# konstin/knn-for-homology

Measured on AMD Instinct MI355X. Metric: queries/sec, flat inner-product kNN, d=1024 fp32, k=100 (recall@k = 1.0: exact flat search), higher is better.
Workload: dtype f32; 1 GPU; BASELINE configs[3]: synthetic 10000000x1024 fp32 flat IP, k=100, 32 queries per step, DB row-sharded over 1 GPU(s); nb_total=10000000, nb_per_gpu=10000000, d=1024, k=100, parallelism=db-row-shard x1, searches_in_flight=1

## Files before the change

### knn-for-homology_amd/csrc/knn355.hip

```cpp
#include <hip/hip_runtime.h>
#include <thread>
#include <type_traits>
#include <stdint.h>
#include <stdio.h>
#include <string.h>
#include <float.h>
#include <math.h>
#include <algorithm>
#include <mutex>
#include <condition_variable>
#include <chrono>
#include <memory>
#include <atomic>
#include <string>
#include <vector>

#include "../../include/knn355.h"
#include "plan.h"

typedef float f32x4 __attribute__((ext_vector_type(4)));
typedef float f32x2 __attribute__((ext_vector_type(2)));
typedef float f32x16 __attribute__((ext_vector_type(16)));
typedef const __attribute__((address_space(1))) f32x4 *gptr4;
typedef __bf16 bf16x8 __attribute__((ext_vector_type(8)));
// ... 868 lines not shown
    "v_cmp_le_f32_e64 %[m0], %[t0], %[e0]\n\t" "v_cmp_le_f32_e64 %[m1], %[t1], %[e1]\n\t" "v_cmp_le_f32_e64 %[m2], %[t2], %[e2]\n\t" "v_cmp_le_f32_e64 %[m3], %[t3], %[e3]\n\t"
#define KNN_P1_TAIL "v_min_u32_e32 %[ad0], %[w], %[dump]\n\t" "v_cndmask_b32_e64 %[u], 0, %[step], %[m0]\n\t" "v_add_u32_e32 %[w], %[w], %[u]\n\t" \
    "v_min_u32_e32 %[ad1], %[w], %[dump]\n\t" "v_cndmask_b32_e64 %[u], 0, %[step], %[m1]\n\t" "v_add_u32_e32 %[w], %[w], %[u]\n\t" \
    "v_min_u32_e32 %[ad2], %[w], %[dump]\n\t" "v_cndmask_b32_e64 %[u], 0, %[step], %[m2]\n\t" "v_add_u32_e32 %[w], %[w], %[u]\n\t" \
    "v_min_u32_e32 %[ad3], %[w], %[dump]\n\t" "v_cndmask_b32_e64 %[u], 0, %[step], %[m3]\n\t" "v_add_u32_e32 %[w], %[w], %[u]\n\t" \
    "v_mov_b32_e32 %[i0], %[idx0]\n\t" "v_mov_b32_e32 %[i1], %[idx1]\n\t" "v_mov_b32_e32 %[i2], %[idx2]\n\t" "v_mov_b32_e32 %[i3], %[idx3]\n\t" \
    "ds_write2_b32 %[ad0], %[t0], %[i0] offset1:1\n\t" "ds_write2_b32 %[ad1], %[t1], %[i1] offset1:1\n\t" "ds_write2_b32 %[ad2], %[t2], %[i2] offset1:1\n\t" "ds_write2_b32 %[ad3], %[t3], %[i3] offset1:1"
#define KNN_P1_OUT_ROW , [e0] "=&v"(e[0]), [e1] "=&v"(e[1]), [e2] "=&v"(e[2]), [e3] "=&v"(e[3])
#define KNN_P1_IN_L2 , [s0] "v"(s0), [s1] "v"(s1), [s2] "v"(s2), [s3] "v"(s3)
#define KNN_P1_IN_THR , [thr] "v"(thr[b])
#define KNN_P1_IN_ROW , [h0] "v"(t2l[sc - c + 0]), [h1] "v"(t2l[sc - c + 1]), [h2] "v"(t2l[sc - c + 2]), [h3] "v"(t2l[sc - c + 3]), [ninf] "v"(ninf), [cok] "s"(cokm[b])
#define KNN_PASS1(head, bound, out_bound, acc_reg, in_l2, in_bound) asm volatile(head bound KNN_P1_TAIL \
    : [t0] "=&v"(t[0]), [t1] "=&v"(t[1]), [t2] "=&v"(t[2]), [t3] "=&v"(t[3]), [ad0] "=&v"(ad[0]), [ad1] "=&v"(ad[1]), [ad2] "=&v"(ad[2]), [ad3] "=&v"(ad[3]), [i0] "=&v"(ix[0]), [i1] "=&v"(ix[1]), [i2] "=&v"(ix[2]), [i3] "=&v"(ix[3]), [m0] "=&s"(mk[0]), [m1] "=&s"(mk[1]), [m2] "=&s"(mk[2]), [m3] "=&s"(mk[3]), [u] "=&v"(u), [w] "+v"(w) out_bound \
    : [a0] acc_reg(a0), [a1] acc_reg(a1), [a2] acc_reg(a2), [a3] acc_reg(a3) in_l2 in_bound, [dump] "v"(dump), [step] "v"(step), [idx0] "n"((sc + 0) | (b << 8)), [idx1] "n"((sc + 1) | (b << 8)), [idx2] "n"((sc + 2) | (b << 8)), [idx3] "n"((sc + 3) | (b << 8)) : "memory")

template <int WM, int WN, int TM, int TN, bool L2, bool NTDB = false, bool SYM = false, bool BF16 = false, int DNQ = 0, int Q16 = 0, bool F16X = false, bool X12 = false>
__global__ __launch_bounds__(256, (TM * TN >= 16 ? 1 : 2)) void flat_scan_kernel(ScanParams p)
{
    if (p.gate) {
        uint32_t any = 0;
        for (int i = 0; i < p.gate_n; i++) any |= p.gate[i];
        if (!any) return;
    }
    constexpr bool DIFF = DNQ > 0;
    static_assert(!F16X || (NTDB && !L2 && !SYM && !BF16 && DNQ == 0 && Q16 == 0 && TN == 1), "the 16-bit prefilter: one query tile, inner product");
    static_assert(!X12 || (F16X && WM == 4 && TM == 2), "the 12-bit row copies: the prefilter's 256-row tile");
    constexpr bool H16 = BF16 || F16X;
    static_assert(WM * WN == 4, "4 waves per workgroup");
    static_assert(!DIFF || (L2 && !SYM && !BF16 && WN == 1 && TN == 1), "the difference build: one 32-query tile, squared L2");
    constexpr bool M16 = Q16 > 0;
    static_assert(!M16 || (NTDB && !SYM && !BF16 && DNQ == 0 && TN == 1), "16-query blocks: plain fp32, one query tile per launch");
    constexpr int DT = WM * TM * 32;
    constexpr int QT = WN * (M16 ? Q16 * 16 : TN * 32);
    constexpr int NB = M16 ? Q16 : TN;
    constexpr int NS = TM * (M16 ? 8 : 16);
    constexpr bool BIGT = TM * TN >= 16;
    constexpr bool SPARSE = !NTDB && !BF16 && DNQ == 0 && Q16 == 0 && WM == 2 && WN == 2 && TM == TN && (TM == 2 || TM == 4);
    constexpr int ROWS = DT + QT;
    constexpr int X12_DB = 24;
    constexpr int NGRP = X12 ? X12_DB + QT / 8 : ROWS / 8;
    constexpr int NI = (NGRP + 3) / 4;
    static_assert(ROWS % 8 == 0, "staging split");
    static_assert(!X12 || NGRP % 4 == 0, "X12: every wave issues whole rounds, the last of them the queries'");
    constexpr int NDBI = X12 ? X12_DB / 4 : DT / 32;
    constexpr int KOFF_DB = X12 ? X12_DB * 256 : 32;
    constexpr int B_OFF = X12 ? X12_DB * 1024 : DT * 128;
    constexpr int STAGE_BYTES = ROWS * 128;
    extern __shared__ __attribute__((aligned(16))) char smem[];
    char *stage0 = smem;
    char *stage1 = smem + STAGE_BYTES;
    const int lds_main = max(max(2 * STAGE_BYTES, p.cap * 8), SYM && TM * TN == 4 ? 73728 : 0);

    const int tid = threadIdx.x;
    const int lane = tid & 63;
// ... 312 lines not shown
                    if constexpr (t < 3) __builtin_amdgcn_sched_group_barrier(0x100, RT + Q16, 0);
                    constexpr int nd = n1 - n0, per = M / (nd + 1);
                    static_assert(per >= 1, "more staging instructions than MFMAs in a sub-step");
                    sched_spread<nd, per>();
                    __builtin_amdgcn_sched_group_barrier(0x008, M - nd * per, 0);
                };
                substep16(std::integral_constant<int, 0>{});
                substep16(std::integral_constant<int, 1>{});
                substep16(std::integral_constant<int, 2>{});
                substep16(std::integral_constant<int, 3>{});
                return;
            }
            if constexpr (X12) {
                typedef uint32_t u32x4 __attribute__((ext_vector_type(4)));
                typedef _Float16 f16x2 __attribute__((ext_vector_type(2)));
                u32x4 hi[TM][2], lo[TM];
                f32x4 bq[4][TN];
#pragma unroll
                for (int a = 0; a < TM; a++) {
                    hi[a][0] = *(const u32x4 *)(A + ((wm * TM + a) * 2 + 0) * 1024 + lane * 16);
                    hi[a][1] = *(const u32x4 *)(A + ((wm * TM + a) * 2 + 1) * 1024 + lane * 16);
                    lo[a] = *(const u32x4 *)(A + DT * 64 + (wm * TM + a) * 1024 + lane * 16);
                }
#pragma unroll
                for (int t = 0; t < 4; t++)
#pragma unroll
                    for (int b = 0; b < TN; b++) bq[t][b] = *(const f32x4 *)(B + ((wn * TN + b) * 32 + li) * 128 + (((2 * t + lh) ^ swz) * 16));
#pragma unroll
                for (int n = 0; n < ND; n++) dma(n);
                const f16x2 bias = {(_Float16)1216.0f, (_Float16)1216.0f}, sixteen = {(_Float16)16.0f, (_Float16)16.0f};
                auto pair = [&](uint32_t hw, uint32_t lw, uint32_t sel) -> uint32_t {
                    const f16x2 ah = __builtin_bit_cast(f16x2, __builtin_amdgcn_perm(0x64646464u, hw, sel)) - bias;
                    const f16x2 al = __builtin_bit_cast(f16x2, __builtin_amdgcn_perm(0x64646464u, lw, sel));
                    return __builtin_bit_cast(uint32_t, __builtin_elementwise_fma(ah, sixteen, al));
                };
#pragma unroll
                for (int t = 0; t < 4; t++) {
#pragma unroll
                    for (int a = 0; a < TM; a++) {
                        const uint32_t h0 = hi[a][t >> 1][2 * (t & 1)], h1 = hi[a][t >> 1][2 * (t & 1) + 1];
                        const uint32_t l0 = lo[a][t] & 0x0F0F0F0Fu, l1 = (lo[a][t] >> 4) & 0x0F0F0F0Fu;
                        const u32x4 fr = {pair(h0, l0, 0x04010400u), pair(h0, l0, 0x04030402u), pair(h1, l1, 0x04010400u), pair(h1, l1, 0x04030402u)};
#pragma unroll
                        for (int b = 0; b < TN; b++)
                            acc[a][b] = __builtin_amdgcn_mfma_f32_32x32x16_f16(__builtin_bit_cast(f16x8, fr), __builtin_bit_cast(f16x8, bq[t][b]), acc[a][b], 0, 0, 0);
                    }
                }
                return;
            }
            f32x4 af[2][TM], bf[2][TN];
            auto frag = [&](int t) {
                const int slot = ((2 * t + lh) ^ swz) * 16;
#pragma unroll
                for (int a = 0; a < TM; a++)
                    af[t & 1][a] = *(const f32x4 *)(A + ((wm * TM + a) * 32 + li) * 128 + slot);
#pragma unroll
                for (int b = 0; b < TN; b++)
// ... 1120 lines not shown
    bool bad;
    const int e = s16_convert(xb + (size_t)r * dp, dp, dp16, xs + (size_t)r * dp16, -128, lane, &nx, &nxp, &nd, &bad);
    if (lane == 0) {
        xexp[r] = (int8_t)e;
        if (bad) {
            atomicOr(&stat[S16_NONFINITE], 1u);
        } else {
            atomicMax(&stat[S16_R], __float_as_uint(s16_up(nd)));
            atomicMax(&stat[S16_XP], __float_as_uint(s16_up(nxp)));
            atomicMax(&stat[S16_X], __float_as_uint(s16_up(nx)));
            atomicMax((int *)&stat[S16_EMAX], e);
        }
    }
}

__global__ __launch_bounds__(256) void scan12_rows_kernel(const float *__restrict__ xb, int dp, int64_t r0, int64_t n, int dp16,
                                                          uint8_t *__restrict__ xs, int8_t *__restrict__ xexp, uint32_t *__restrict__ stat)
{
    const int lane = threadIdx.x & 63;
    const int64_t r = r0 + (int64_t)blockIdx.x * 4 + (threadIdx.x >> 6);
    if (r >= r0 + n) return;
    const float *x = xb + (size_t)r * dp;
    float mx = 0.0f;
    bool nf = false;
    for (int i = lane; i < dp; i += 64) {
        const float v = x[i];
        nf |= !isfinite(v);
        mx = fmaxf(mx, fabsf(v));
    }
    for (int o = 32; o > 0; o >>= 1) mx = fmaxf(mx, __shfl_xor(mx, o, 64));
    const bool bad = __ballot(nf) != 0ull;
    int e = (mx > 0.0f && isfinite(mx)) ? ilogbf(mx) - 10 : 0;
    e = max(e, -128);
    const int KT = dp16 / 64, rt = (int)(r & 255), li = rt & 31, wa = rt >> 5;
    uint8_t *tile = xs + (size_t)(r >> 8) * KT * 24576;
    double sx = 0.0, sxp = 0.0, sd = 0.0;
    for (int g = lane; g < dp16 / 8; g += 64) {
        const int ks = g >> 3, t = (g >> 1) & 3, lh = g & 1;
        uint32_t hw[2] = {0u, 0u}, lw = 0u;
        for (int j = 0; j < 8; j++) {
            const int i = 8 * g + j;
            const float v = i < dp ? x[i] : 0.0f;
            float nv = rintf(ldexpf(v, -e));
            nv = fminf(fmaxf(nv, -2047.0f), 2047.0f);
            const int ni = nv == nv ? (int)nv : 0;
            const uint32_t u = (uint32_t)(ni + 2048);
            hw[j >> 2] |= (u >> 4) << (8 * (j & 3));
            lw |= (u & 15u) << (8 * (j & 3) + 4 * (j >> 2));
            const double xp = ldexp((double)ni, e), dv = (double)v;
            sx += dv * dv;
            sxp += xp * xp;
            sd += (dv - xp) * (dv - xp);
        }
        uint8_t *ksp = tile + (size_t)ks * 24576;
        *(uint2 *)(ksp + (wa * 2 + (t >> 1)) * 1024 + (lh * 32 + li) * 16 + (t & 1) * 8) = make_uint2(hw[0], hw[1]);
        *(uint32_t *)(ksp + 16384 + wa * 1024 + (lh * 32 + li) * 16 + t * 4) = lw;
    }
    for (int o = 32; o > 0; o >>= 1) {
        sx += __shfl_xor(sx, o, 64);
        sxp += __shfl_xor(sxp, o, 64);
        sd += __shfl_xor(sd, o, 64);
    }
    if (lane == 0) {
        xexp[r] = (int8_t)e;
        if (bad) {
            atomicOr(&stat[S16_NONFINITE], 1u);
        } else {
            atomicMax(&stat[S16_R], __float_as_uint(s16_up(sqrt(sd))));
            atomicMax(&stat[S16_XP], __float_as_uint(s16_up(sqrt(sxp))));
            atomicMax(&stat[S16_X], __float_as_uint(s16_up(sqrt(sx))));
            atomicMax((int *)&stat[S16_EMAX], e);
// ... 370 lines not shown
};

struct knn_index_s {
    int d = 0, dp = 0, metric = 0, device = 0;
    int num_cus = 256;
    int64_t ntotal = 0, cap_rows = 0;
    bool is_view = false;
    std::shared_ptr<std::atomic<int64_t>> storage_gen = std::make_shared<std::atomic<int64_t>>(0);
    int64_t view_gen = 0;
    float *xb = nullptr;
    bool approx16 = false;
    bool keep16 = false;
    DevBuf xb16, ws_q16;
    int scan16 = 0;
    int s16_fmt = 16;
    std::shared_ptr<std::atomic<bool>> s16_ok = std::make_shared<std::atomic<bool>>(false);
    int dp16 = 0;
    DevBuf s16_rows_buf, s16_exp_buf, s16_stat_buf;
    const _Float16 *s16_rows = nullptr;
    const int8_t *s16_exp = nullptr;
    const uint32_t *s16_stat = nullptr;
    std::string s16_note;
    DevBuf ws_q16x, ws_s16q, ws_s16ak, ws_s16ok, ws_s16stat;
    bool last_s16_used = false;
    int last_s16_fmt = 0;
    int s16_pieces = 0;
    float *yn = nullptr;
    size_t xb_bytes = 0, yn_bytes = 0;
    hipStream_t stream = nullptr;
    hipEvent_t done = nullptr;
// ... 210 lines not shown
    (void)hipEventCreateWithFlags(&h->done, hipEventDisableTiming);
    *out = h;
    return 0;
}

static void free_index_buffers(knn_index_s *h)
{
    if (!h->is_view) h->storage_gen->fetch_add(1);
    if (h->xb && !h->is_view) g_pool.give(h->xb, h->xb_bytes, h->device);
    if (h->yn && !h->is_view) g_pool.give(h->yn, h->yn_bytes, h->device);
    if (!h->is_view) {
        h->s16_rows_buf.release();
        h->s16_exp_buf.release();
        h->s16_stat_buf.release();
        if (h->scan16 == 2) h->scan16 = 1;
    }
    h->s16_rows = nullptr;
    h->s16_exp = nullptr;
    h->s16_stat = nullptr;
    if (!h->is_view) h->s16_ok->store(false);
    h->xb = nullptr;
    h->yn = nullptr;
    h->ntotal = 0;
    h->cap_rows = 0;
}

extern "C" void knn_free(knn_handle h)
{
    if (!h) return;
    if (hipSetDevice(h->device) == hipSuccess) {
// ... 88 lines not shown
    if (h->xb16.bytes < need) {
        if (h->xb16.ensure(need)) return set_err(KNN_ERR_HIP, "add: out of device memory (bf16 rows)");
        n += r0;
        r0 = 0;
    }
    const int64_t total = n * h->dp;
    const unsigned grid = (unsigned)std::min<int64_t>((total / 4 + 255) / 256, 65535);
    hipLaunchKernelGGL(to_bf16_kernel, dim3(grid), dim3(256), 0, s, h->xb + (size_t)r0 * h->dp, total, (__bf16 *)h->xb16.p + (size_t)r0 * h->dp);
    HIP_TRY(hipGetLastError());
    return 0;
}

static int scan16_sync_rows(knn_index_s *h, int64_t r0, int64_t n, hipStream_t s)
{
    if (h->scan16 != 1 || h->is_view) return 0;
    const size_t need = h->s16_fmt == 12 ? (size_t)((h->cap_rows + 255) / 256) * (h->dp16 / 64) * 24576 : (size_t)h->cap_rows * h->dp16 * 2;
    if (h->cap_rows > 0 && (h->s16_rows_buf.bytes < need || h->s16_exp_buf.bytes < (size_t)h->cap_rows || !h->s16_stat_buf.p)) {
        HIP_TRY(hipStreamSynchronize(s));
        if (h->s16_rows_buf.p || h->s16_exp_buf.p) {
            h->storage_gen->fetch_add(1);
            (void)hipDeviceSynchronize();
        }
        if (h->s16_rows_buf.ensure(need) || h->s16_exp_buf.ensure((size_t)h->cap_rows) || h->s16_stat_buf.ensure(S16_NSTAT * 4)) {
            h->s16_rows_buf.release();
            h->s16_exp_buf.release();
            h->s16_stat_buf.release();
            h->s16_rows = nullptr;
            h->s16_exp = nullptr;
            h->s16_stat = nullptr;
            h->s16_ok->store(false);
            h->scan16 = 2;
            h->s16_note = "dropped: no device memory for the row copies";
            return 0;
        }
        n += r0;
        r0 = 0;
    }
    if (n <= 0) return 0;
    h->s16_rows = (const _Float16 *)h->s16_rows_buf.p;
    h->s16_exp = (const int8_t *)h->s16_exp_buf.p;
    h->s16_stat = (const uint32_t *)h->s16_stat_buf.p;
    uint32_t init[S16_NSTAT] = {0u, 0u, 0u, 0x80000000u, 0u, 0u, 0u, 0u};
    if (r0 == 0) HIP_TRY(hipMemcpyAsync(h->s16_stat_buf.p, init, sizeof init, hipMemcpyHostToDevice, s));
    if (h->s16_fmt == 12)
        hipLaunchKernelGGL(scan12_rows_kernel, dim3((unsigned)((n + 3) / 4)), dim3(256), 0, s, h->xb, h->dp, r0, n, h->dp16,
                           (uint8_t *)h->s16_rows_buf.p, (int8_t *)h->s16_exp_buf.p, (uint32_t *)h->s16_stat_buf.p);
    else
        hipLaunchKernelGGL(scan16_rows_kernel, dim3((unsigned)((n + 3) / 4)), dim3(256), 0, s, h->xb, h->dp, r0, n, h->dp16,
                           (_Float16 *)h->s16_rows_buf.p, (int8_t *)h->s16_exp_buf.p, (uint32_t *)h->s16_stat_buf.p);
    HIP_TRY(hipGetLastError());
    uint32_t nonfinite = 0;
    HIP_TRY(hipMemcpyAsync(&nonfinite, (const uint32_t *)h->s16_stat_buf.p + S16_NONFINITE, 4, hipMemcpyDeviceToHost, s));
    HIP_TRY(hipStreamSynchronize(s));
    h->s16_ok->store(nonfinite == 0);
    h->s16_note = nonfinite ? "off: a row holds a value that is not finite" : "on";
    return 0;
}

static int flat_set_approx16(knn_index_s *h)
{
// ... 199 lines not shown
}

static ScanKernel pick_scan_kernel(int qt, bool l2, bool approx16, bool one_qtile, int diff_width, int pass_mode, int s16_fmt = 16)
{
    if (const char *why = scan_kernel_illegal(qt, l2, approx16, one_qtile, pass_mode)) {
        set_err(KNN_ERR_INVALID, why);
        return nullptr;
    }
    switch (qt) {
    case 256: return l2 ? flat_scan_kernel<2, 2, 4, 4, true, false> : flat_scan_kernel<2, 2, 4, 4, false, false>;
    case 128: return scan_build<2, 2, 2, 2>(l2, approx16, one_qtile);
    case 96: return l2 ? flat_scan_kernel<2, 2, 2, 1, true, true, false, false, 0, 3> : flat_scan_kernel<2, 2, 2, 1, false, true, false, false, 0, 3>;
    case 48: return l2 ? flat_scan_kernel<4, 1, 2, 1, true, true, false, false, 0, 3> : flat_scan_kernel<4, 1, 2, 1, false, true, false, false, 0, 3>;
    case 64: return scan_build<2, 2, 2, 1>(l2, approx16, one_qtile);
    }
    if (pass_mode == 1 && s16_fmt == 12) return flat_scan_kernel<4, 1, 2, 1, false, true, false, false, 0, 0, true, true>;
    if (pass_mode == 1) return flat_scan_kernel<4, 1, 2, 1, false, true, false, false, 0, 0, true>;
    switch (diff_width) {
    case 0: break;
    case 8: return flat_scan_kernel<4, 1, 2, 1, true, true, false, false, 8>;
    case 12: return flat_scan_kernel<4, 1, 2, 1, true, true, false, false, 12>;
    case 16: return flat_scan_kernel<4, 1, 2, 1, true, true, false, false, 16>;
    default: return flat_scan_kernel<4, 1, 2, 1, true, true, false, false, 20>;
    }
    return scan_build<4, 1, 2, 1>(l2, approx16, one_qtile);
}

static ScanKernel pick_sym_kernel(int ts, bool l2)
{
    if (ts == 128) return l2 ? flat_scan_kernel<2, 2, 2, 2, true, false, true> : flat_scan_kernel<2, 2, 2, 2, false, false, true>;
    return l2 ? flat_scan_kernel<2, 2, 4, 4, true, false, true> : flat_scan_kernel<2, 2, 4, 4, false, false, true>;
// ... 156 lines not shown
    }
    if (pl.npairs && sstride) {
        if (lb.pair_ctr.ensure(((size_t)pl.npairs + 1) * 4, h->done, s)) return set_err(KNN_ERR_HIP, "search: out of device memory");
        HIP_TRY(hipMemsetD32Async((hipDeviceptr_t)lb.pair_ctr.p, 2, (size_t)pl.npairs, s));
        HIP_TRY(hipMemsetD32Async((hipDeviceptr_t)((uint32_t *)lb.pair_ctr.p + pl.npairs), 0, 1, s));
    }
    if (h->ws_lists.ensure((size_t)pl.grid * pl.qt * pl.cap * 8, h->done, s)) return set_err(KNN_ERR_HIP, "search: out of device memory (candidate lists)");
    ScanParams p = {};
    p.xb = h->xb; p.yn = h->yn; p.xq = q_dev; p.xn = xn;
    p.nb = nb; p.nq = nq; p.dp = h->dp; p.k = k; p.cap = pl.cap;
    if (h->approx16) {
        p.xb = (const float *)h->xb16.p;
        p.dp = h->dp / 2;
    }
    if (pass.mode == 1) {
        if (h->s16_fmt == 12 && (row_mul != 1 || sstride)) return set_err(KNN_ERR_INVALID, "search: the 12-bit row copies cannot serve a strided view");
        p.xb = (const float *)h->s16_rows;
        p.dp = h->dp16 / 2;
        p.xexp = h->s16_exp;
        p.qexp = pass.qexp;
    }
    p.gate = pass.gate;
    p.gate_n = pass.gate_n;
    p.nqtiles = pl.nqtiles; p.nchunks = pl.nchunks; p.tiles_base = pl.tiles_base; p.tiles_rem = pl.tiles_rem;
    p.lists = (uint64_t *)h->ws_lists.p; p.gthr = gthr;
    p.qlist = qlist; p.qcnt = qcnt; p.qcap = qcap;
    p.id_base = id_base;
    p.row_mul = row_mul;
    p.vshift = sstride ? svshift : vshift;
    p.skip_mask = sstride ? sstride - 1 : -1;
    p.kslot = plan.kslot;
// ... 25 lines not shown
        if (g_trace_buf.ensure((size_t)pl.grid * 128 * 8)) return set_err(KNN_ERR_HIP, "trace: out of device memory");
        HIP_TRY(hipMemsetAsync(g_trace_buf.p, 0, (size_t)pl.grid * 128 * 8, s));
        p.trace = (unsigned long long *)g_trace_buf.p;
        p.ablate = getenv("KNN355_ABLATE") ? atoi(getenv("KNN355_ABLATE")) : 0;
        g_trace_grid = pl.grid;
    }
#endif
    if (top && (rc = open_timed_launch(h, s))) return rc;
    const ScanKernel kern = pick_scan_kernel(pl.qt, h->metric == KNN_METRIC_L2, h->approx16, pl.nqtiles == 1, pl.diff ? diff_build_width(nq) : 0, pass.mode, h->s16_fmt);
    if (!kern) return KNN_ERR_INVALID;
    rc = scan_lds_opt_in(kern, pl.lds);
    if (!rc) rc = launch_scan(kern, p, pl.grid, pl.lds, s);
    if (rc) return rc;
    if (top) {
        HIP_TRY(hipEventRecord(h->ev1, s));
        h->last_kernel = pass.mode == 1 ? std::string(pl.name) + (h->s16_fmt == 12 ? "_x12" : "_f16x") : std::string(pl.name); h->last_qt = pl.qt; h->last_dt = pl.dt; h->last_chunks = pl.nchunks; h->last_grid = pl.grid;
        h->last_seed_stride = pub_rounds ? -pub_rounds * pub_m : sstride;
        h->last_seed_stat = seed_stat ? plan.seed_j : 0;
        h->last_sample_rows = sstride ? view_rows(nb, sstride, p.vshift) : 0;
    }
    SelectParams sp = {};
    sp.in = qlist; sp.in_stride = qcap; sp.cnt = qcnt; sp.cap = qcap;
    sp.n_expect = select_expect_n(plan, nb, k, sstride ? view_rows(nb, sstride, p.vshift) : 0);
    sp.nq = nq; sp.k = k; sp.metric = h->metric;
    sp.out_keys = out.keys; sp.out_stride = out.keys ? out.keys_stride : 0; sp.out_fill = out.keys_fill;
    sp.D = out.D; sp.I = out.I;
    sp.seed_cnt = out.seed_cnt; sp.seed_gthr = out.seed_gthr; sp.seed_qthr = out.seed_qthr; sp.seed_j = out.seed_j; sp.seed_stat = out.seed_stat;
    sp.seed_nslots = out.seed_nslots;
    sp.qthr = qthr; sp.fail = (int *)h->ws_flag.p;
    sp.gate = pass.gate; sp.gate_n = pass.gate_n; sp.gate_count = pass.gate_count;
    if (reset_sig && out.seed_cnt == nullptr) {
// ... 672 lines not shown
extern "C" int knn_flat_reserve(knn_handle h, int64_t nrows)
{
    if (!h) return set_err(KNN_ERR_INVALID, "reserve: null handle");
    if (nrows < 0 || nrows > 0xFFFFFFF0ll) return set_err(KNN_ERR_INVALID, "reserve: bad row count");
    std::lock_guard<std::mutex> lk(h->mu);
    if (h->is_view) return set_err(KNN_ERR_INVALID, "reserve: a view is read-only");
    HIP_TRY(hipSetDevice(h->device));
    if (nrows <= h->cap_rows) return 0;
    if (int rc = move_storage(h, nrows, "reserve")) return rc;
    return scan16_sync_rows(h, h->ntotal, 0, h->stream);
}

extern "C" int knn_flat_set_scan16(knn_handle h, int32_t mode)
{
    if (!h) return set_err(KNN_ERR_INVALID, "set_scan16: null handle");
    if (mode != 0 && mode != 1 && mode != 2) return set_err(KNN_ERR_INVALID, "set_scan16: mode must be 0, 1 or 2");
    std::lock_guard<std::mutex> lk(h->mu);
    if (h->is_view) return set_err(KNN_ERR_INVALID, "set_scan16: a view uses its parent's setting");
    if (mode && (h->approx16 || h->keep16)) return set_err(KNN_ERR_UNSUPPORTED, "set_scan16: not for an index that keeps bf16 copies (HNSW)");
    if (h->ntotal != 0) return set_err(KNN_ERR_INVALID, "set_scan16: the index already holds rows");
    const char *env = getenv("KNN355_SCAN16");
    if (mode && env && strcmp(env, "0") == 0) mode = 0;
    const char *fenv = getenv("KNN355_SCAN_FORMAT");
    if (mode == 2 && fenv && strcmp(fenv, "16") == 0) mode = 1;
    h->scan16 = mode ? 1 : 0;
    h->s16_fmt = mode == 2 ? 12 : 16;
    h->dp16 = round_up(h->d, 64);
    h->s16_note = mode ? "on" : "off";
    return 0;
}

extern "C" int knn_last_scan16_info(knn_handle h, int32_t *used, int32_t *candidates_max, int64_t *fallbacks)
{
    if (!h) return set_err(KNN_ERR_INVALID, "null handle");
    std::lock_guard<std::mutex> lk(h->mu);
    uint32_t st[2] = {0u, 0u};
    if (h->ws_s16stat.p) {
        HIP_TRY(hipSetDevice(h->device));
        HIP_TRY(hipDeviceSynchronize());
        HIP_TRY(hipMemcpy(st, h->ws_s16stat.p, sizeof st, hipMemcpyDeviceToHost));
    }
// ... 414 lines not shown
```

### knn-for-homology_amd/csrc/plan.h

```cpp
#pragma once
#include <stddef.h>
#include <stdint.h>
#include <stdlib.h>
#include <math.h>
#include <algorithm>
#include <vector>

#include "../../include/knn355.h"

struct PlanCtx {
    int metric = KNN_METRIC_INNER_PRODUCT;
    bool approx16 = false;
    int flags = 0, force_qt = 0, force_chunks = 0;
    int num_cus = 256;
    int64_t batch_nq = 0;
    int pub_rounds_force = 0;
    int64_t ntotal = 0;
    int s16_fmt = 16;
};

static inline int64_t view_rows(int64_t n, int row_mul, int vshift)
{
    const int64_t B = (int64_t)1 << vshift, span = B * row_mul;
    if (n <= 0) return 0;
// ... 142 lines not shown
{
    if (S < 64 || N <= 0 || k >= N) return -1;
    const double pr = (double)k / (double)N, eps = 1e-9;
    const double lp = log(pr), lq = log1p(-pr);
    double cdf = 0.0;
    const int64_t jmax = std::min<int64_t>(S, k);
    for (int64_t i = 0; i <= jmax; i++) {
        if (1.0 - cdf <= eps) return i >= 1 ? (int)i : 1;
        cdf += exp(lgamma((double)S + 1.0) - lgamma((double)i + 1.0) - lgamma((double)(S - i) + 1.0) + (double)i * lp + (double)(S - i) * lq);
    }
    return -1;
}

static int s16_kprime(int k, int fmt = 16)
{
    if (fmt == 12) return std::min(KNN_WAVE_SELECT_MAX_K, std::max(3 * k, k + 128));
    return std::min(KNN_WAVE_SELECT_MAX_K, std::max(2 * k, k + 64));
}

static bool s16_eligible(const PlanCtx &c, int pass_mode, int64_t nb, int64_t nq, int k, int row_mul, int level, int dp, int fmt = 16)
{
    if (pass_mode || level != 0 || row_mul != 1) return false;
    if (c.metric != KNN_METRIC_INNER_PRODUCT || c.approx16 || (c.flags & KNN_TUNE_NO_SCAN16)) return false;
    if (nq < 1 || nq > 32 || (c.force_qt != 0 && c.force_qt != 32) || s16_kprime(k, fmt) <= k) return false;
    if ((size_t)dp * 4 + 64 > 65536) return false;
    return nb >= (1 << 18) || (c.flags & KNN_TUNE_SCAN16_ANY_NB);
}

struct SearchPlan {
    ScanPlan pl;
    int sstride;
    int svshift;
    int seed_j, seed_stat, k_sample;
    int pub_rounds, pub_m;
    int kslot, qcap;
    double expect_n;
    int pool_tiles;
    bool sparse_epi, cu_turn;
};
// ... 54 lines not shown
        if (c.pub_rounds_force > 0 && (int64_t)c.pub_rounds_force * pl.nchunks <= 2048 && c.pub_rounds_force < pl.tiles_base &&
            (int64_t)c.pub_rounds_force * pl.nchunks >= (int64_t)k + 32)
            pub_rounds = c.pub_rounds_force;
    }
    if (!pub_rounds && pub_shape && !c.pub_rounds_force && nb >= 16 * (int64_t)k && k <= KNN_WAVE_SELECT_MAX_K) {
        const int wm = (pl.qt == 32 || pl.qt == 48) ? 4 : 2;
        for (int r = 2; r >= 1; r--) {
            const int64_t P = (int64_t)r * wm * pl.nchunks;
            if (P <= 4096 && P >= (int64_t)k + k / 4 + 32 && r < pl.tiles_base) {
                pub_rounds = r;
                pub_m = wm;
            }
        }
    }
    if (pass_mode == 2 && !pub_rounds) sstride = 0;
    if (pass_mode == 1 && c.s16_fmt == 12 && !pub_rounds) sstride = 0;
    if (pub_rounds) {
        sstride = 0;
        expect_n = 2.0 * (double)k * (double)nb / ((double)pub_rounds * pl.nchunks * pl.dt) + 2.0 * k + 64;
        if (pub_m > 1) {
            const double P = (double)pub_rounds * pub_m * pl.nchunks;
            expect_n = 1.3 * (-P * log(1.0 - (double)k / P)) * (double)nb / ((double)pub_rounds * pl.nchunks * pl.dt) + 2.0 * k + 64;
        }
    }
    if (!sstride && !pub_rounds) {
        PlanOpts final_plan;
        final_plan.seeded = level > 0; final_plan.allow_pairs = allow_pairs && level == 0; final_plan.allow_big = allow_big;
        make_plan(c, nb, nq, k, final_plan, pl);
    }
    int kslot = knn_kslot(k);
    if (pl.chunk_rows == pl.dt && pl.dt > kslot && pl.dt <= pl.cap - pl.dt && k <= KNN_WAVE_SELECT_MAX_K) kslot = pl.dt;
// ... 459 lines not shown
```

### knn-for-homology_amd/csrc/plan_check.cpp

```cpp
#include "plan.h"

#include <stdarg.h>
#include <stdio.h>
#include <string.h>
#include <set>
#include <string>
#include <tuple>

static const int MAX_LEVELS = 8;

static PlanCtx make_ctx(int64_t nb, int64_t nq, int metric, int flags, int force_qt, int force_chunks, int64_t batch, bool approx16)
{
    PlanCtx c;
    c.metric = metric;
    c.approx16 = approx16;
    c.flags = flags & ~KNN_TUNE_PUB_ROUNDS_MASK;
    c.pub_rounds_force = (flags & KNN_TUNE_PUB_ROUNDS_MASK) >> KNN_TUNE_PUB_ROUNDS_SHIFT;
    c.force_qt = force_qt;
    c.force_chunks = force_chunks;
    c.num_cus = 256;
    c.batch_nq = batch > 0 ? std::max(nq, batch) : nq;
    c.ntotal = nb;
    return c;
}
// ... 437 lines not shown
        starts.push_back(starts[0]);
        stops.push_back(stops[0]);
        for (int64_t chunk_rows : {(int64_t)1, (int64_t)2, (int64_t)7, (int64_t)64, (int64_t)119, (int64_t)120, rows - 1, rows, rows + 1, (int64_t)1 << 40})
            if (chunk_rows >= 1) check_pool_chunks(starts, stops, chunk_rows);
    }
}

static int run_s16()
{
    long long nb, nq;
    int k, flags;
    while (scanf("%lld %lld %d %d", &nb, &nq, &k, &flags) == 4) {
        const PlanCtx c = make_ctx(nb, nq, KNN_METRIC_INNER_PRODUCT, flags, 0, 0, 0, false);
        printf("%lld %lld %d %d: fp16 kprime %d eligible %d, 12-bit kprime %d eligible %d\n", nb, nq, k, flags, s16_kprime(k, 16),
               (int)s16_eligible(c, 0, nb, nq, k, 1, 0, 1024, 16), s16_kprime(k, 12), (int)s16_eligible(c, 0, nb, nq, k, 1, 0, 1024, 12));
    }
    return 0;
}

static int run_sweep()
{
    const int64_t nbs[] = {1, 255, 256, 257, 1023, 4096, 8192, 16385, 1 << 15, 1 << 18, (1 << 18) + 1, 1250000, 10000000, 2147483647};
    const int64_t nqs[] = {1, 8, 19, 20, 32, 33, 48, 49, 64, 65, 96, 97, 128, 129, 256, 384, 640, 16384, 24576, 24577, 200000};
    const int ks[] = {1, 10, 100, 301, 1000, 1400, 1401, 2048};
    const int flagset[] = {0, KNN_TUNE_NO_POOL, KNN_TUNE_NO_PAIRS, KNN_TUNE_NO_SEED, KNN_TUNE_EXACT_SEED, KNN_TUNE_NORM_L2, KNN_TUNE_ALWAYS_RESET,
                           KNN_TUNE_STAT_SEED, KNN_TUNE_NO_TURNS, KNN_TUNE_NO_STAT_SEED, KNN_TUNE_NO_SYM, KNN_TUNE_NO_TILE_MIN_SEED,
                           1 << KNN_TUNE_PUB_ROUNDS_SHIFT, 2 << KNN_TUNE_PUB_ROUNDS_SHIFT, KNN_TUNE_NO_REMAINDER_SPLIT, KNN_TUNE_NO_Q16,
                           KNN_TUNE_NO_BIG_TILE, KNN_TUNE_BIG_TILE, KNN_TUNE_NO_SCAN16, KNN_TUNE_SCAN16_ANY_NB};
    const int qts[] = {0, 32, 48, 64, 96, 128, 256};
    for (int64_t nb : nbs)
// ... 28 lines not shown
                for (int key_bytes : {2, 4, 8})
                    for (int outs = 0; outs < 8; outs++) check_rank(rows, k, limit, key_bytes, outs);
        }
    sweep_pool();
    sweep_kde();
    printf("plan_check sweep: %lld plans checked, %lld broken\n", g_checked, g_broken);
    return g_broken ? 1 : 0;
}

int main(int argc, char **argv)
{
    if (argc == 2 && !strcmp(argv[1], "cases")) return run_cases();
    if (argc == 2 && !strcmp(argv[1], "sym")) return run_sym();
    if (argc == 2 && !strcmp(argv[1], "range")) return run_range();
    if (argc == 2 && !strcmp(argv[1], "s16")) return run_s16();
    if (argc == 2 && !strcmp(argv[1], "rank")) return run_rank();
    if (argc == 2 && !strcmp(argv[1], "pool")) return run_pool();
    if (argc == 2 && !strcmp(argv[1], "poolchunks")) return run_poolchunks();
    if (argc == 2 && !strcmp(argv[1], "kde")) return run_kde();
    if (argc == 2 && !strcmp(argv[1], "sweep")) return run_sweep();
    fprintf(stderr, "usage: plan_check cases|sym|range|s16|rank|pool|poolchunks|kde < lines | plan_check sweep\n");
    return 2;
}
```

Before: 12750 queries/s.

## Add 10-bit packed row copies for the prefilter scan, auto-selected on large indexes

Adds a 10-bit packed format for the database copies used by the 16-bit prefilter pass, alongside the existing 12-bit one. A byte high part plus 2-bit low parts cut each k-step tile from 24 KiB to 20 KiB. The point is to reduce the memory bandwidth of the bandwidth-bound scan. Mode 2 now picks 10-bit automatically when rows×dims reach 2^33 values. The cost is coarser quantisation, so the candidate count k' grows to max(8k, k+256), which adds selection work and exact rescoring.

```diff
diff --git a/knn-for-homology_amd/csrc/knn355.hip b/knn-for-homology_amd/csrc/knn355.hip
--- a/knn-for-homology_amd/csrc/knn355.hip
+++ b/knn-for-homology_amd/csrc/knn355.hip
@@ -906,7 +906,7 @@
     : [t0] "=&v"(t[0]), [t1] "=&v"(t[1]), [t2] "=&v"(t[2]), [t3] "=&v"(t[3]), [ad0] "=&v"(ad[0]), [ad1] "=&v"(ad[1]), [ad2] "=&v"(ad[2]), [ad3] "=&v"(ad[3]), [i0] "=&v"(ix[0]), [i1] "=&v"(ix[1]), [i2] "=&v"(ix[2]), [i3] "=&v"(ix[3]), [m0] "=&s"(mk[0]), [m1] "=&s"(mk[1]), [m2] "=&s"(mk[2]), [m3] "=&s"(mk[3]), [u] "=&v"(u), [w] "+v"(w) out_bound \
     : [a0] acc_reg(a0), [a1] acc_reg(a1), [a2] acc_reg(a2), [a3] acc_reg(a3) in_l2 in_bound, [dump] "v"(dump), [step] "v"(step), [idx0] "n"((sc + 0) | (b << 8)), [idx1] "n"((sc + 1) | (b << 8)), [idx2] "n"((sc + 2) | (b << 8)), [idx3] "n"((sc + 3) | (b << 8)) : "memory")
 
-template <int WM, int WN, int TM, int TN, bool L2, bool NTDB = false, bool SYM = false, bool BF16 = false, int DNQ = 0, int Q16 = 0, bool F16X = false, bool X12 = false>
+template <int WM, int WN, int TM, int TN, bool L2, bool NTDB = false, bool SYM = false, bool BF16 = false, int DNQ = 0, int Q16 = 0, bool F16X = false, int XW = 0>
 __global__ __launch_bounds__(256, (TM * TN >= 16 ? 1 : 2)) void flat_scan_kernel(ScanParams p)
 {
     if (p.gate) {
@@ -916,7 +916,9 @@
     }
     constexpr bool DIFF = DNQ > 0;
     static_assert(!F16X || (NTDB && !L2 && !SYM && !BF16 && DNQ == 0 && Q16 == 0 && TN == 1), "the 16-bit prefilter: one query tile, inner product");
-    static_assert(!X12 || (F16X && WM == 4 && TM == 2), "the 12-bit row copies: the prefilter's 256-row tile");
+    static_assert(XW == 0 || XW == 12 || XW == 10, "the packed row copies' width: 12 or 10 bits (0: none)");
+    constexpr bool X12 = XW != 0;
+    static_assert(!X12 || (F16X && WM == 4 && TM == 2), "the packed row copies: the prefilter's 256-row tile");
     constexpr bool H16 = BF16 || F16X;
     static_assert(WM * WN == 4, "4 waves per workgroup");
     static_assert(!DIFF || (L2 && !SYM && !BF16 && WN == 1 && TN == 1), "the difference build: one 32-query tile, squared L2");
@@ -929,7 +931,7 @@
     constexpr bool BIGT = TM * TN >= 16;
     constexpr bool SPARSE = !NTDB && !BF16 && DNQ == 0 && Q16 == 0 && WM == 2 && WN == 2 && TM == TN && (TM == 2 || TM == 4);
     constexpr int ROWS = DT + QT;
-    constexpr int X12_DB = 24;
+    constexpr int X12_DB = XW == 10 ? 20 : 24;
     constexpr int NGRP = X12 ? X12_DB + QT / 8 : ROWS / 8;
     constexpr int NI = (NGRP + 3) / 4;
     static_assert(ROWS % 8 == 0, "staging split");
@@ -1272,24 +1274,26 @@
             if constexpr (X12) {
                 typedef uint32_t u32x4 __attribute__((ext_vector_type(4)));
                 typedef _Float16 f16x2 __attribute__((ext_vector_type(2)));
-                u32x4 hi[TM][2], lo[TM];
+                u32x4 hi[TM][2], lo[XW == 10 ? 1 : TM];
                 f32x4 bq[4][TN];
 #pragma unroll
                 for (int a = 0; a < TM; a++) {
                     hi[a][0] = *(const u32x4 *)(A + ((wm * TM + a) * 2 + 0) * 1024 + lane * 16);
                     hi[a][1] = *(const u32x4 *)(A + ((wm * TM + a) * 2 + 1) * 1024 + lane * 16);
-                    lo[a] = *(const u32x4 *)(A + DT * 64 + (wm * TM + a) * 1024 + lane * 16);
+                    if constexpr (XW != 10) lo[a] = *(const u32x4 *)(A + DT * 64 + (wm * TM + a) * 1024 + lane * 16);
                 }
+                if constexpr (XW == 10) lo[0] = *(const u32x4 *)(A + DT * 64 + wm * 1024 + lane * 16);
 #pragma unroll
                 for (int t = 0; t < 4; t++)
 #pragma unroll
                     for (int b = 0; b < TN; b++) bq[t][b] = *(const f32x4 *)(B + ((wn * TN + b) * 32 + li) * 128 + (((2 * t + lh) ^ swz) * 16));
 #pragma unroll
                 for (int n = 0; n < ND; n++) dma(n);
-                const f16x2 bias = {(_Float16)1216.0f, (_Float16)1216.0f}, sixteen = {(_Float16)16.0f, (_Float16)16.0f};
-                auto pair = [&](uint32_t hw, uint32_t lw, uint32_t sel) -> uint32_t {
+                constexpr float BIAS = XW == 10 ? 1408.0f : 1216.0f, STEP = XW == 10 ? 4.0f : 16.0f;
+                const f16x2 bias = {(_Float16)BIAS, (_Float16)BIAS}, sixteen = {(_Float16)STEP, (_Float16)STEP};
+                auto pair = [&](uint32_t hw, uint32_t lw, uint32_t sel, uint32_t lsel) -> uint32_t {
                     const f16x2 ah = __builtin_bit_cast(f16x2, __builtin_amdgcn_perm(0x64646464u, hw, sel)) - bias;
-                    const f16x2 al = __builtin_bit_cast(f16x2, __builtin_amdgcn_perm(0x64646464u, lw, sel));
+                    const f16x2 al = __builtin_bit_cast(f16x2, __builtin_amdgcn_perm(0x64646464u, lw, lsel));
                     return __builtin_bit_cast(uint32_t, __builtin_elementwise_fma(ah, sixteen, al));
                 };
 #pragma unroll
@@ -1297,8 +1301,16 @@
 #pragma unroll
                     for (int a = 0; a < TM; a++) {
                         const uint32_t h0 = hi[a][t >> 1][2 * (t & 1)], h1 = hi[a][t >> 1][2 * (t & 1) + 1];
-                        const uint32_t l0 = lo[a][t] & 0x0F0F0F0Fu, l1 = (lo[a][t] >> 4) & 0x0F0F0F0Fu;
-                        const u32x4 fr = {pair(h0, l0, 0x04010400u), pair(h0, l0, 0x04030402u), pair(h1, l1, 0x04010400u), pair(h1, l1, 0x04030402u)};
+                        u32x4 fr;
+                        if constexpr (XW == 10) {
+                            const uint32_t w = lo[0][2 * a + (t >> 1)], ls = (t & 1) ? 0x04030402u : 0x04010400u;
+                            fr = u32x4{pair(h0, w & 0x03030303u, 0x04010400u, ls), pair(h0, (w >> 2) & 0x03030303u, 0x04030402u, ls),
+                                       pair(h1, (w >> 4) & 0x03030303u, 0x04010400u, ls), pair(h1, (w >> 6) & 0x03030303u, 0x04030402u, ls)};
+                        } else {
+                            const uint32_t l0 = lo[a][t] & 0x0F0F0F0Fu, l1 = (lo[a][t] >> 4) & 0x0F0F0F0Fu;
+                            fr = u32x4{pair(h0, l0, 0x04010400u, 0x04010400u), pair(h0, l0, 0x04030402u, 0x04030402u),
+                                       pair(h1, l1, 0x04010400u, 0x04010400u), pair(h1, l1, 0x04030402u, 0x04030402u)};
+                        }
 #pragma unroll
                         for (int b = 0; b < TN; b++)
                             acc[a][b] = __builtin_amdgcn_mfma_f32_32x32x16_f16(__builtin_bit_cast(f16x8, fr), __builtin_bit_cast(f16x8, bq[t][b]), acc[a][b], 0, 0, 0);
@@ -2449,7 +2461,8 @@
     }
 }
 
-__global__ __launch_bounds__(256) void scan12_rows_kernel(const float *__restrict__ xb, int dp, int64_t r0, int64_t n, int dp16,
+template <int XW>
+__global__ __launch_bounds__(256) void scan_packed_rows_kernel(const float *__restrict__ xb, int dp, int64_t r0, int64_t n, int dp16,
                                                           uint8_t *__restrict__ xs, int8_t *__restrict__ xexp, uint32_t *__restrict__ stat)
 {
     const int lane = threadIdx.x & 63;
@@ -2465,10 +2478,12 @@
     }
     for (int o = 32; o > 0; o >>= 1) mx = fmaxf(mx, __shfl_xor(mx, o, 64));
     const bool bad = __ballot(nf) != 0ull;
-    int e = (mx > 0.0f && isfinite(mx)) ? ilogbf(mx) - 10 : 0;
+    static_assert(XW == 12 || XW == 10, "12- or 10-bit copies");
+    constexpr int LIM = (1 << (XW - 1)) - 1, LB = XW - 8, KSB = 16384 + 2048 * LB;
+    int e = (mx > 0.0f && isfinite(mx)) ? ilogbf(mx) - (XW - 2) : 0;
     e = max(e, -128);
     const int KT = dp16 / 64, rt = (int)(r & 255), li = rt & 31, wa = rt >> 5;
-    uint8_t *tile = xs + (size_t)(r >> 8) * KT * 24576;
+    uint8_t *tile = xs + (size_t)(r >> 8) * KT * KSB;
     double sx = 0.0, sxp = 0.0, sd = 0.0;
     for (int g = lane; g < dp16 / 8; g += 64) {
         const int ks = g >> 3, t = (g >> 1) & 3, lh = g & 1;
@@ -2477,19 +2492,21 @@
             const int i = 8 * g + j;
             const float v = i < dp ? x[i] : 0.0f;
             float nv = rintf(ldexpf(v, -e));
-            nv = fminf(fmaxf(nv, -2047.0f), 2047.0f);
+            nv = fminf(fmaxf(nv, -(float)LIM), (float)LIM);
             const int ni = nv == nv ? (int)nv : 0;
-            const uint32_t u = (uint32_t)(ni + 2048);
-            hw[j >> 2] |= (u >> 4) << (8 * (j & 3));
-            lw |= (u & 15u) << (8 * (j & 3) + 4 * (j >> 2));
+            const uint32_t u = (uint32_t)(ni + LIM + 1);
+            hw[j >> 2] |= (u >> LB) << (8 * (j & 3));
+            if constexpr (XW == 10) lw |= (u & 3u) << (8 * (j & 1) + 2 * (j >> 1));
+            else lw |= (u & 15u) << (8 * (j & 3) + 4 * (j >> 2));
             const double xp = ldexp((double)ni, e), dv = (double)v;
             sx += dv * dv;
             sxp += xp * xp;
             sd += (dv - xp) * (dv - xp);
         }
-        uint8_t *ksp = tile + (size_t)ks * 24576;
+        uint8_t *ksp = tile + (size_t)ks * KSB;
         *(uint2 *)(ksp + (wa * 2 + (t >> 1)) * 1024 + (lh * 32 + li) * 16 + (t & 1) * 8) = make_uint2(hw[0], hw[1]);
-        *(uint32_t *)(ksp + 16384 + wa * 1024 + (lh * 32 + li) * 16 + t * 4) = lw;
+        if constexpr (XW == 10) *(uint16_t *)(ksp + 16384 + (wa >> 1) * 1024 + (lh * 32 + li) * 16 + (wa & 1) * 8 + t * 2) = (uint16_t)lw;
+        else *(uint32_t *)(ksp + 16384 + wa * 1024 + (lh * 32 + li) * 16 + t * 4) = lw;
     }
     for (int o = 32; o > 0; o >>= 1) {
         sx += __shfl_xor(sx, o, 64);
@@ -2890,6 +2907,9 @@
     DevBuf xb16, ws_q16;
     int scan16 = 0;
     int s16_fmt = 16;
+    bool s16_auto = false;
+    bool s16_chosen = false;
+    int64_t s16_min_values = S16_SCAN10_MIN_VALUES;
     std::shared_ptr<std::atomic<bool>> s16_ok = std::make_shared<std::atomic<bool>>(false);
     int dp16 = 0;
     DevBuf s16_rows_buf, s16_exp_buf, s16_stat_buf;
@@ -3130,6 +3150,7 @@
         h->s16_exp_buf.release();
         h->s16_stat_buf.release();
         if (h->scan16 == 2) h->scan16 = 1;
+        h->s16_chosen = false;
     }
     h->s16_rows = nullptr;
     h->s16_exp = nullptr;
@@ -3248,7 +3269,11 @@
 static int scan16_sync_rows(knn_index_s *h, int64_t r0, int64_t n, hipStream_t s)
 {
     if (h->scan16 != 1 || h->is_view) return 0;
-    const size_t need = h->s16_fmt == 12 ? (size_t)((h->cap_rows + 255) / 256) * (h->dp16 / 64) * 24576 : (size_t)h->cap_rows * h->dp16 * 2;
+    if (h->s16_auto && !h->s16_chosen && h->cap_rows > 0) {
+        h->s16_fmt = s16_packed_width(h->cap_rows, h->dp16, h->s16_min_values);
+        h->s16_chosen = true;
+    }
+    const size_t need = h->s16_fmt != 16 ? (size_t)((h->cap_rows + 255) / 256) * (h->dp16 / 64) * s16_tile_kstep_bytes(h->s16_fmt) : (size_t)h->cap_rows * h->dp16 * 2;
     if (h->cap_rows > 0 && (h->s16_rows_buf.bytes < need || h->s16_exp_buf.bytes < (size_t)h->cap_rows || !h->s16_stat_buf.p)) {
         HIP_TRY(hipStreamSynchronize(s));
         if (h->s16_rows_buf.p || h->s16_exp_buf.p) {
@@ -3276,8 +3301,11 @@
     h->s16_stat = (const uint32_t *)h->s16_stat_buf.p;
     uint32_t init[S16_NSTAT] = {0u, 0u, 0u, 0x80000000u, 0u, 0u, 0u, 0u};
     if (r0 == 0) HIP_TRY(hipMemcpyAsync(h->s16_stat_buf.p, init, sizeof init, hipMemcpyHostToDevice, s));
-    if (h->s16_fmt == 12)
-        hipLaunchKernelGGL(scan12_rows_kernel, dim3((unsigned)((n + 3) / 4)), dim3(256), 0, s, h->xb, h->dp, r0, n, h->dp16,
+    if (h->s16_fmt == 10)
+        hipLaunchKernelGGL(scan_packed_rows_kernel<10>, dim3((unsigned)((n + 3) / 4)), dim3(256), 0, s, h->xb, h->dp, r0, n, h->dp16,
+                           (uint8_t *)h->s16_rows_buf.p, (int8_t *)h->s16_exp_buf.p, (uint32_t *)h->s16_stat_buf.p);
+    else if (h->s16_fmt == 12)
+        hipLaunchKernelGGL(scan_packed_rows_kernel<12>, dim3((unsigned)((n + 3) / 4)), dim3(256), 0, s, h->xb, h->dp, r0, n, h->dp16,
                            (uint8_t *)h->s16_rows_buf.p, (int8_t *)h->s16_exp_buf.p, (uint32_t *)h->s16_stat_buf.p);
     else
         hipLaunchKernelGGL(scan16_rows_kernel, dim3((unsigned)((n + 3) / 4)), dim3(256), 0, s, h->xb, h->dp, r0, n, h->dp16,
@@ -3507,7 +3535,8 @@
     case 48: return l2 ? flat_scan_kernel<4, 1, 2, 1, true, true, false, false, 0, 3> : flat_scan_kernel<4, 1, 2, 1, false, true, false, false, 0, 3>;
     case 64: return scan_build<2, 2, 2, 1>(l2, approx16, one_qtile);
     }
-    if (pass_mode == 1 && s16_fmt == 12) return flat_scan_kernel<4, 1, 2, 1, false, true, false, false, 0, 0, true, true>;
+    if (pass_mode == 1 && s16_fmt == 12) return flat_scan_kernel<4, 1, 2, 1, false, true, false, false, 0, 0, true, 12>;
+    if (pass_mode == 1 && s16_fmt == 10) return flat_scan_kernel<4, 1, 2, 1, false, true, false, false, 0, 0, true, 10>;
     if (pass_mode == 1) return flat_scan_kernel<4, 1, 2, 1, false, true, false, false, 0, 0, true>;
     switch (diff_width) {
     case 0: break;
@@ -3694,7 +3723,7 @@
         p.dp = h->dp / 2;
     }
     if (pass.mode == 1) {
-        if (h->s16_fmt == 12 && (row_mul != 1 || sstride)) return set_err(KNN_ERR_INVALID, "search: the 12-bit row copies cannot serve a strided view");
+        if (h->s16_fmt != 16 && (row_mul != 1 || sstride)) return set_err(KNN_ERR_INVALID, "search: the packed row copies cannot serve a strided view");
         p.xb = (const float *)h->s16_rows;
         p.dp = h->dp16 / 2;
         p.xexp = h->s16_exp;
@@ -3750,7 +3779,7 @@
     if (rc) return rc;
     if (top) {
         HIP_TRY(hipEventRecord(h->ev1, s));
-        h->last_kernel = pass.mode == 1 ? std::string(pl.name) + (h->s16_fmt == 12 ? "_x12" : "_f16x") : std::string(pl.name); h->last_qt = pl.qt; h->last_dt = pl.dt; h->last_chunks = pl.nchunks; h->last_grid = pl.grid;
+        h->last_kernel = pass.mode == 1 ? std::string(pl.name) + (h->s16_fmt == 12 ? "_x12" : h->s16_fmt == 10 ? "_x10" : "_f16x") : std::string(pl.name); h->last_qt = pl.qt; h->last_dt = pl.dt; h->last_chunks = pl.nchunks; h->last_grid = pl.grid;
         h->last_seed_stride = pub_rounds ? -pub_rounds * pub_m : sstride;
         h->last_seed_stat = seed_stat ? plan.seed_j : 0;
         h->last_sample_rows = sstride ? view_rows(nb, sstride, p.vshift) : 0;
@@ -4453,7 +4482,7 @@
 extern "C" int knn_flat_set_scan16(knn_handle h, int32_t mode)
 {
     if (!h) return set_err(KNN_ERR_INVALID, "set_scan16: null handle");
-    if (mode != 0 && mode != 1 && mode != 2) return set_err(KNN_ERR_INVALID, "set_scan16: mode must be 0, 1 or 2");
+    if (mode < 0 || mode > 4) return set_err(KNN_ERR_INVALID, "set_scan16: mode must be 0, 1, 2, 3 or 4");
     std::lock_guard<std::mutex> lk(h->mu);
     if (h->is_view) return set_err(KNN_ERR_INVALID, "set_scan16: a view uses its parent's setting");
     if (mode && (h->approx16 || h->keep16)) return set_err(KNN_ERR_UNSUPPORTED, "set_scan16: not for an index that keeps bf16 copies (HNSW)");
@@ -4461,9 +4490,19 @@
     const char *env = getenv("KNN355_SCAN16");
     if (mode && env && strcmp(env, "0") == 0) mode = 0;
     const char *fenv = getenv("KNN355_SCAN_FORMAT");
-    if (mode == 2 && fenv && strcmp(fenv, "16") == 0) mode = 1;
+    if (mode >= 2 && fenv && strcmp(fenv, "16") == 0) mode = 1;
+    if (mode >= 2 && fenv && strcmp(fenv, "12") == 0) mode = 4;
+    if (mode >= 2 && fenv && strcmp(fenv, "10") == 0) mode = 3;
     h->scan16 = mode ? 1 : 0;
-    h->s16_fmt = mode == 2 ? 12 : 16;
+    h->s16_fmt = mode == 3 ? 10 : mode >= 2 ? 12 : 16;
+    h->s16_auto = mode == 2;
+    h->s16_chosen = false;
+    h->s16_min_values = S16_SCAN10_MIN_VALUES;
+    if (const char *menv = getenv("KNN355_SCAN10_MIN_VALUES")) {
+        char *end = nullptr;
+        const long long v = strtoll(menv, &end, 10);
+        if (end != menv && *end == 0 && v >= 0) h->s16_min_values = v;
+    }
     h->dp16 = round_up(h->d, 64);
     h->s16_note = mode ? "on" : "off";
     return 0;
diff --git a/knn-for-homology_amd/csrc/plan.h b/knn-for-homology_amd/csrc/plan.h
--- a/knn-for-homology_amd/csrc/plan.h
+++ b/knn-for-homology_amd/csrc/plan.h
@@ -180,15 +180,22 @@
 
 static int s16_kprime(int k, int fmt = 16)
 {
+    if (fmt == 10) return std::min(KNN_WAVE_SELECT_MAX_K, std::max(8 * k, k + 256));
     if (fmt == 12) return std::min(KNN_WAVE_SELECT_MAX_K, std::max(3 * k, k + 128));
     return std::min(KNN_WAVE_SELECT_MAX_K, std::max(2 * k, k + 64));
 }
+
+static size_t s16_tile_kstep_bytes(int fmt) { return fmt == 10 ? 20480 : 24576; }
+
+constexpr int64_t S16_SCAN10_MIN_VALUES = (int64_t)1 << 33;
+static int s16_packed_width(int64_t cap_rows, int dp16, int64_t min_values) { return cap_rows * (int64_t)dp16 >= min_values ? 10 : 12; }
 
 static bool s16_eligible(const PlanCtx &c, int pass_mode, int64_t nb, int64_t nq, int k, int row_mul, int level, int dp, int fmt = 16)
 {
     if (pass_mode || level != 0 || row_mul != 1) return false;
     if (c.metric != KNN_METRIC_INNER_PRODUCT || c.approx16 || (c.flags & KNN_TUNE_NO_SCAN16)) return false;
     if (nq < 1 || nq > 32 || (c.force_qt != 0 && c.force_qt != 32) || s16_kprime(k, fmt) <= k) return false;
+    if (fmt == 10 && 8 * (int64_t)k > KNN_WAVE_SELECT_MAX_K) return false;
     if ((size_t)dp * 4 + 64 > 65536) return false;
     return nb >= (1 << 18) || (c.flags & KNN_TUNE_SCAN16_ANY_NB);
 }
@@ -273,7 +280,7 @@
         }
     }
     if (pass_mode == 2 && !pub_rounds) sstride = 0;
-    if (pass_mode == 1 && c.s16_fmt == 12 && !pub_rounds) sstride = 0;
+    if (pass_mode == 1 && c.s16_fmt != 16 && !pub_rounds) sstride = 0;
     if (pub_rounds) {
         sstride = 0;
         expect_n = 2.0 * (double)k * (double)nb / ((double)pub_rounds * pl.nchunks * pl.dt) + 2.0 * k + 64;
diff --git a/knn-for-homology_amd/csrc/plan_check.cpp b/knn-for-homology_amd/csrc/plan_check.cpp
--- a/knn-for-homology_amd/csrc/plan_check.cpp
+++ b/knn-for-homology_amd/csrc/plan_check.cpp
@@ -475,6 +475,19 @@
         const PlanCtx c = make_ctx(nb, nq, KNN_METRIC_INNER_PRODUCT, flags, 0, 0, 0, false);
         printf("%lld %lld %d %d: fp16 kprime %d eligible %d, 12-bit kprime %d eligible %d\n", nb, nq, k, flags, s16_kprime(k, 16),
                (int)s16_eligible(c, 0, nb, nq, k, 1, 0, 1024, 16), s16_kprime(k, 12), (int)s16_eligible(c, 0, nb, nq, k, 1, 0, 1024, 12));
+    }
+    return 0;
+}
+
+static int run_s10()
+{
+    long long nb, nq, cap_rows, min_values;
+    int k, flags, dp16;
+    while (scanf("%lld %lld %d %d %lld %d %lld", &nb, &nq, &k, &flags, &cap_rows, &dp16, &min_values) == 7) {
+        const PlanCtx c = make_ctx(nb, nq, KNN_METRIC_INNER_PRODUCT, flags, 0, 0, 0, false);
+        printf("%lld %lld %d %d: 10-bit kprime %d eligible %d, width %d of %lld x %d\n", nb, nq, k, flags, s16_kprime(k, 10),
+               (int)s16_eligible(c, 0, nb, nq, k, 1, 0, 1024, 10), s16_packed_width(cap_rows, dp16, min_values < 0 ? S16_SCAN10_MIN_VALUES : min_values),
+               cap_rows, dp16);
     }
     return 0;
 }
@@ -533,11 +546,12 @@
     if (argc == 2 && !strcmp(argv[1], "sym")) return run_sym();
     if (argc == 2 && !strcmp(argv[1], "range")) return run_range();
     if (argc == 2 && !strcmp(argv[1], "s16")) return run_s16();
+    if (argc == 2 && !strcmp(argv[1], "s10")) return run_s10();
     if (argc == 2 && !strcmp(argv[1], "rank")) return run_rank();
     if (argc == 2 && !strcmp(argv[1], "pool")) return run_pool();
     if (argc == 2 && !strcmp(argv[1], "poolchunks")) return run_poolchunks();
     if (argc == 2 && !strcmp(argv[1], "kde")) return run_kde();
     if (argc == 2 && !strcmp(argv[1], "sweep")) return run_sweep();
-    fprintf(stderr, "usage: plan_check cases|sym|range|s16|rank|pool|poolchunks|kde < lines | plan_check sweep\n");
+    fprintf(stderr, "usage: plan_check cases|sym|range|s16|s10|rank|pool|poolchunks|kde < lines | plan_check sweep\n");
     return 2;
 }
```

New measurement: 11840 queries/s. 7.2% lower.
